# GuyTevet/motion-diffusion-model

Hardware: NVIDIA H100
Metric: motions/sec (higher is better)
Workload: dtype fp16 operands / fp32 accumulate (in/out projections hi-lo split)

## Files before the change

### motion-diffusion-model_b200/csrc/engine.cu

```cuda
#include <cuda.h>
#include <cuda_fp16.h>
#include <cuda_runtime.h>

#include <cmath>
#include <cstdarg>
#include <cstdio>
#include <cstring>
#include <map>
#include <string>
#include <vector>

#include "../../include/b200mdm.h"
#include "attention_tc.cuh"
#include "epilogues.cuh"
#include "gemm.cuh"
#include "gemm_ln.cuh"
#include "postprocess.cuh"
#include "kernels.cuh"

using namespace b200;

static thread_local char g_err[512] = "";
static int fail(int code, const char* fmt, ...) {
  va_list ap;
  va_start(ap, fmt);
  vsnprintf(g_err, sizeof(g_err), fmt, ap);
  va_end(ap);
  return code;
}
#define CUDA_TRY(expr)                                                                               \
  do {                                                                                               \
    cudaError_t _e = (expr);                                                                         \
    if (_e != cudaSuccess)                                                                           \
      return fail(B200MDM_ECUDA, "%s failed: %s (%s:%d)", #expr, cudaGetErrorString(_e), __FILE__, __LINE__); \
  } while (0)
#define TRY(expr)            \
  do {                       \
    int _r = (expr);         \
    if (_r != B200MDM_OK) return _r; \
  } while (0)

typedef CUresult (*EncodeTiledFn)(CUtensorMap*, CUtensorMapDataType, cuuint32_t, void*, const cuuint64_t*,
                                  const cuuint64_t*, const cuuint32_t*, const cuuint32_t*, CUtensorMapInterleave,
                                  CUtensorMapSwizzle, CUtensorMapL2promotion, CUtensorMapFloatOOBfill);
static EncodeTiledFn g_encode = nullptr;
static int resolve_driver() {
  if (g_encode) return B200MDM_OK;
  void* fn = nullptr;
  cudaDriverEntryPointQueryResult qres;
// ... 129 lines not shown
  std::vector<int> h_kv, h_action;
  std::vector<unsigned char> h_mask;
  bool dec = false;
  int ctx = 0, s_off = 1;
  int kw = 1;
  const unsigned char* inpaint_mask = nullptr;
  const float* inpaint_motion = nullptr;
  unsigned long long noise_seed = 0;
  long long noise_sample_base = 0;
  StepState* state = nullptr;
  cudaStream_t work = nullptr;
  cudaEvent_t ev_in = nullptr, ev_out = nullptr;
  long long launches = 0;
};

template <class T>
static int dalloc(T** p, size_t n, bool zero = false) {
  CUDA_TRY(cudaMalloc(reinterpret_cast<void**>(p), n * sizeof(T)));
  if (zero) CUDA_TRY(cudaMemset(*p, 0, n * sizeof(T)));
  return B200MDM_OK;
}
template <class T>
static void dfree(T*& p) {
  if (p) cudaFree(p);
  p = nullptr;
}

template <int BN, class Epi, bool RES = false>
static int set_gemm_attr() {
  CUDA_TRY(cudaFuncSetAttribute(gemm_f16_wgmma<BN, Epi, RES>, cudaFuncAttributeMaxDynamicSharedMemorySize,
                                GemmSmem<BN, Epi, RES>::TOTAL));
  return B200MDM_OK;
}
template <int KEYS>
static int set_attention_attr() {
  CUDA_TRY(cudaFuncSetAttribute(attention_tc_kernel<KEYS, false>, cudaFuncAttributeMaxDynamicSharedMemorySize,
                                AttnTcSmem::total(KEYS)));
  CUDA_TRY(cudaFuncSetAttribute(attention_tc_kernel<KEYS, true>, cudaFuncAttributeMaxDynamicSharedMemorySize,
                                AttnTcSmem::total(KEYS)));
  return B200MDM_OK;
}
static int init_kernel_attrs() {
  static unsigned long long done_mask = 0;
  int dev = 0;
  CUDA_TRY(cudaGetDevice(&dev));
  if (dev < 64 && ((done_mask >> dev) & 1ull)) return B200MDM_OK;
  TRY((set_gemm_attr<128, EpiBiasF16<false>>()));
  TRY((set_gemm_attr<128, EpiBiasF16<true>>()));
  TRY((set_gemm_attr<256, EpiBiasF16<false>>()));
  TRY((set_gemm_attr<256, EpiBiasF16<true>>()));
  TRY((set_gemm_attr<64, EpiBiasF16<false>, true>()));
  TRY((set_gemm_attr<64, EpiBiasF16<true>, true>()));
  TRY((set_gemm_attr<128, EpiBiasF16Wide<true>>()));
  TRY((set_gemm_attr<128, EpiBiasF16Global>()));
  CUDA_TRY(cudaFuncSetAttribute(gemm_resid_ln_cluster, cudaFuncAttributeMaxDynamicSharedMemorySize, GemmLnSmem::TOTAL));
  TRY((set_gemm_attr<128, EpiEmbed>()));
  TRY((set_gemm_attr<96, EpiOutStep>()));
  TRY((set_attention_attr<64>()));
  TRY((set_attention_attr<208>()));
  TRY((set_attention_attr<256>()));
  if (dev < 64) done_mask |= 1ull << dev;
  return B200MDM_OK;
}

static bool g_pdl_now = false;
static bool pdl_enabled() {
  static int v = -1;
  if (v < 0) {
    const char* e = getenv("B200MDM_PDL");
    v = (e && e[0] == '0') ? 0 : 1;
  }
  return v == 1;
}
struct PdlScope {
  PdlScope() { g_pdl_now = pdl_enabled(); }
  ~PdlScope() { g_pdl_now = false; }
};
template <class... KArgs, class... Args>
static cudaError_t launch_k(void (*kern)(KArgs...), dim3 grid, dim3 block, size_t smem, cudaStream_t s, Args&&... args) {
  cudaLaunchConfig_t cfg;
  memset(&cfg, 0, sizeof(cfg));
  cfg.gridDim = grid;
  cfg.blockDim = block;
  cfg.dynamicSmemBytes = smem;
  cfg.stream = s;
  cudaLaunchAttribute at[1];
  at[0].id = cudaLaunchAttributeProgrammaticStreamSerialization;
  at[0].val.programmaticStreamSerializationAllowed = 1;
  cfg.attrs = at;
  cfg.numAttrs = g_pdl_now ? 1 : 0;
  return cudaLaunchKernelEx(&cfg, kern, static_cast<KArgs>(std::forward<Args>(args))...);
}

template <int BN, class Epi, class = void> struct epi_unstaged : std::false_type {};
template <int BN, class Epi> struct epi_unstaged<BN, Epi, std::enable_if_t<Epi::UNSTAGED>> : std::true_type {};

template <int BN, class Epi>
static int launch_gemm(const CUtensorMap& a, const CUtensorMap& b, const CUtensorMap& c, int M, int N, int K,
                       const typename Epi::Params& p, cudaStream_t s, int num_sms) {
  if (!epi_unstaged<BN, Epi>::value && N * 4 > GEMM_BIAS_BYTES)
    return fail(B200MDM_ENOTIMPL, "GEMM epilogue vectors are staged for N <= %d", GEMM_BIAS_BYTES / 4);
  const int tiles = ((M + GEMM_BLOCK_M - 1) / GEMM_BLOCK_M) * ((N + BN - 1) / BN);
  const int grid = tiles < num_sms ? tiles : num_sms;
  CUDA_TRY(launch_k(gemm_f16_wgmma<BN, Epi>, dim3(grid), dim3(GEMM_THREADS), GemmSmem<BN, Epi>::TOTAL, s, a, b, c, M, N, K, p));
  return B200MDM_OK;
}
template <int BN, class Epi>
static int launch_gemm_resident(const CUtensorMap& a, const CUtensorMap& b, const CUtensorMap& c, int M, int N, int K,
                                const typename Epi::Params& p, cudaStream_t s, int num_sms) {
  const int tiles_n = (N + BN - 1) / BN;
  const int tiles = ((M + GEMM_BLOCK_M - 1) / GEMM_BLOCK_M) * tiles_n;
  const int grid = tiles < num_sms ? tiles : num_sms;
  if (K > GEMM_RES_KB_MAX * GEMM_BLOCK_K || tiles_n > grid || N * 4 > GEMM_BIAS_BYTES)
    return fail(B200MDM_ENOTIMPL, "W-resident GEMM needs K <= %d and N <= %d", GEMM_RES_KB_MAX * GEMM_BLOCK_K, grid * BN);
  CUDA_TRY(launch_k(gemm_f16_wgmma<BN, Epi, true>, dim3(grid), dim3(GEMM_THREADS), GemmSmem<BN, Epi, true>::TOTAL, s, a, b, c, M, N, K, p));
  return B200MDM_OK;
}
template <bool GELU>
static int launch_gemm_bias(const CUtensorMap& a, const CUtensorMap& b, const CUtensorMap& c, int M, int N, int K,
                            const float* bias, cudaStream_t s, int num_sms) {
  typename EpiBiasF16<GELU>::Params p{bias};
  return launch_gemm<128, EpiBiasF16<GELU>>(a, b, c, M, N, K, p, s, num_sms);
}

static int launch_gemm_resid_ln(const CUtensorMap& a, const CUtensorMap& w256, const CUtensorMap& hres, int M, int K,
                                const float* bias, const float* gamma, const float* beta, cudaStream_t s, int num_sms) {
  const int tiles = (M + GEMM_BLOCK_M - 1) / GEMM_BLOCK_M;
  const int max_clusters = num_sms / 2;
  const int clusters = tiles < max_clusters ? tiles : max_clusters;
  GemmLnParams lp{bias, gamma, beta, 1e-5f};
  CUDA_TRY(launch_k(gemm_resid_ln_cluster, dim3(2 * clusters), dim3(GLN_THREADS), GemmLnSmem::TOTAL, s, a, w256, hres, M, K, lp));
  return B200MDM_OK;
}

static int make_attention_kv_map(CUtensorMap* m, const void* qkv, int n_samples, int S, int ld) {
  return make_map_3d(m, qkv, n_samples, S, ld, ld, atc_keys(S));
}
template <int KEYS>
static cudaError_t launch_attention_keys(const CUtensorMap& map_kv, const __half* qkv, __half* out, const int* kvlen,
                                         dim3 grid, int S, int d, float scale_log2, cudaStream_t s, bool wide) {
  return launch_k(wide ? attention_tc_kernel<KEYS, true> : attention_tc_kernel<KEYS, false>, grid, dim3(ATC_THREADS),
                  AttnTcSmem::total(KEYS), s, map_kv, qkv, out, kvlen, S, d, scale_log2);
}
static int launch_attention_tc(const CUtensorMap& map_kv, const __half* qkv, __half* out, const int* kvlen, int n_samples,
                               int S, int d, int H, cudaStream_t s, bool wide = false) {
  if (d != H * ATC_DH) return fail(B200MDM_ENOTIMPL, "attention: head_dim must be 128");
  if (S > ATC_MAX_KEYS) return fail(B200MDM_ENOTIMPL, "attention: at most %d tokens per sample", ATC_MAX_KEYS);
  const float scale_log2 = 1.4426950408889634f / sqrtf(static_cast<float>(ATC_DH));
  const int tiles = (S + ATC_QROWS - 1) / ATC_QROWS;
  const dim3 grid(H, n_samples, (tiles + ATC_TILES_PER_CTA - 1) / ATC_TILES_PER_CTA);
  const int keys = atc_keys(S);
  if (keys == 64) CUDA_TRY(launch_attention_keys<64>(map_kv, qkv, out, kvlen, grid, S, d, scale_log2, s, wide));
  else if (keys == 208) CUDA_TRY(launch_attention_keys<208>(map_kv, qkv, out, kvlen, grid, S, d, scale_log2, s, wide));
  else CUDA_TRY(launch_attention_keys<256>(map_kv, qkv, out, kvlen, grid, S, d, scale_log2, s, wide));
  return B200MDM_OK;
// ... 651 lines not shown

static int enqueue_forward(b200mdm_engine* e, const StepArgs& a, cudaStream_t s, int* n_kernels) {
  const int d = e->d, ff = e->ff, B = e->B, T = e->T, S = e->S, JF = e->JF, Kp = e->Kp_in;
  int nk = 0;
  PdlScope pdl_scope;
  if (a.philox) {
    const long long quads = (static_cast<long long>(JF) * T + 3) / 4 * B;
    const int blocks = static_cast<int>(quads / 256 + 1 < 1184 ? quads / 256 + 1 : 1184);
    CUDA_TRY(launch_k(philox_normal_kernel, dim3(blocks), dim3(256), 0, s, e->eps_buf, B, static_cast<long long>(JF) * T,
                      0ull, 0ll, 0u, e->state));
    ++nk;
  }
  {
    dim3 grid((T + 31) / 32, (JF + 31) / 32, B), block(32, 8);
    CUDA_TRY(launch_k(pack_input_kernel, grid, block, 0, s, a.x_in, e->xin16, B, JF, T, S, Kp, 3 * Kp, e->s_off));
    ++nk;
  }
  {
    EpiEmbed::Params p;
    p.res_c = e->m_res_c; p.res_u = e->m_res_u;
    p.pe_bias = e->pe_bias;
    p.S = S; p.d = d; p.halves = e->halves;
    TRY((launch_gemm<128, EpiEmbed>(e->m_xin, e->m_win, e->m_xin, e->MB, d, 3 * Kp, p, s, e->num_sms)));
    ++nk;
  }
  const float* target_g = e->target_set ? e->tgt_g : nullptr;
  if (!e->dec) {
    CUDA_TRY(launch_k(tok0_rows_kernel, dim3(e->Bp), dim3(128), 0, s, e->hres, e->condproj, e->temb_table, e->pe,
                      a.explicit_t ? e->tvec : nullptr, e->tmap, e->state, target_g, B, S, d, e->cfg.temb_rows));
  } else {
    CUDA_TRY(launch_k(mem_build_kernel, dim3(e->Mt, e->Bp), dim3(128), 0, s, e->mem16, e->memproj, e->temb_table,
                      a.explicit_t ? e->tvec : nullptr, e->tmap, e->state, target_g, B, e->Mt, d, e->cfg.temb_rows));
    EpiBiasF16Global::Params p{e->bkv_all};
    TRY((launch_gemm<128, EpiBiasF16Global>(e->m_mem, e->m_wkv_all, e->m_kvc_st, e->Bp * e->Mt, e->L * 2 * d, d, p, s, e->num_sms)));
    ++nk;
  }
  ++nk;
  const int kw = e->kw;
  const bool wide = kw == 2;
  for (int l = 0; l < e->L; ++l) {
    const LayerW& w = e->layers[l];
    if (B200_SKIP(1)) {
      ++nk;
    } else {
      {
        TRY((launch_gemm_bias<false>(e->m_h16, w.m_wqkv, e->m_qkv_st, e->M, 3 * d, d, w.bqkv, s, e->num_sms)));
      }
      TRY(launch_attention_tc(e->m_qkv_kv, e->qkv16, e->att16, e->kvlen, e->Bp, S, d, e->H, s, wide));
    }
    if (!B200_SKIP(2)) TRY(launch_gemm_resid_ln(e->m_att, w.m_wo_256, e->m_hres, e->M, kw * d, w.bo, w.g1, w.be1, s, e->num_sms));
    if (e->dec) {
      TRY((launch_gemm_bias<false>(e->m_h16, w.m_wq_c, e->m_qc_st, e->M, d, d, w.bq_c, s, e->num_sms)));
      {
        const float sl2 = 1.4426950408889634f / sqrtf(128.0f);
        const dim3 cg(e->H, e->Bp), cb(128);
        const __half* kvl = e->kvc16 + static_cast<size_t>(l) * 2 * d;
        const int ldkv = e->L * 2 * d;
        if (e->Mt <= 16)
          CUDA_TRY(launch_k(cross_attention_kernel<2>, cg, cb, 0, s, e->qc16, kvl, e->memmask, e->att16, S, e->Mt, d, ldkv, sl2));
        else if (e->Mt <= 32)
          CUDA_TRY(launch_k(cross_attention_kernel<4>, cg, cb, 0, s, e->qc16, kvl, e->memmask, e->att16, S, e->Mt, d, ldkv, sl2));
        else
          CUDA_TRY(launch_k(cross_attention_kernel<8>, cg, cb, 0, s, e->qc16, kvl, e->memmask, e->att16, S, e->Mt, d, ldkv, sl2));
      }
      TRY(launch_gemm_resid_ln(e->m_att, w.m_wo_c_256, e->m_hres, e->M, d, w.bo_c, w.g2, w.be2, s, e->num_sms));
      nk += 3;
    }
    if (wide) {
      EpiBiasF16Wide<true>::Params p{w.b1, ff};
      TRY((launch_gemm<128, EpiBiasF16Wide<true>>(e->m_h16, w.m_w1, e->m_ffn_st, e->M, ff, kw * d, p, s, e->num_sms)));
    } else if (!B200_SKIP(4)) {
      TRY((launch_gemm_bias<true>(e->m_h16, w.m_w1, e->m_ffn_st, e->M, ff, d, w.b1, s, e->num_sms)));
    }
    if (!B200_SKIP(8)) TRY(launch_gemm_resid_ln(e->m_ffn, w.m_w2_256, e->m_hres, e->M, kw * ff, w.b2, e->dec ? w.g3 : w.g2,
                             e->dec ? w.be3 : w.be2, s, e->num_sms));
    nk += 5;
  }
  CUDA_TRY(launch_k(blend_split_kernel, dim3((B * T + 7) / 8), dim3(256), 0, s, e->hres, e->g16, e->scale, B, S, T, e->s_off, d,
                    e->halves));
  ++nk;
  {
    EpiOutStep::Params p;
    p.bias = e->b_out;
    p.x_t = a.x_in;
    p.noise = a.noise;
    p.x_out = a.x_out;
    p.pred_xstart = a.pred;
    p.inpaint_mask = e->inpaint_mask;
    p.inpaint_motion = e->inpaint_motion;
    p.sched = e->sched;
    p.state = e->state;
    p.noise_batch_stride = a.const_noise ? 0 : static_cast<long long>(JF) * T;
    p.B = B; p.S = T; p.T = T; p.J = JF; p.mode = a.mode;
    p.s_off = 0;
    p.clip_denoised = a.clip;
    TRY((launch_gemm<96, EpiOutStep>(e->m_g16, e->m_wout, e->m_g16, B * T, e->N_out_pad, 3 * d, p, s, e->num_sms)));
    ++nk;
  }
  *n_kernels = nk;
  return B200MDM_OK;
}

static int check_ready(b200mdm_engine* e, bool need_sched) {
// ... 157 lines not shown
  CUDA_TRY(cudaGetLastError());
  return B200MDM_OK;
}

extern "C" int b200mdm_q_sample(b200mdm_engine* e, float sqrt_ac, float sqrt_1mac, const float* x_start_dev,
                                const float* noise_dev, float* out_dev, int64_t n, void* stream) {
  if (!e || !noise_dev || !out_dev || n <= 0) return fail(B200MDM_EINVAL, "bad argument");
  q_sample_kernel<<<592, 256, 0, static_cast<cudaStream_t>(stream)>>>(out_dev, x_start_dev, noise_dev, sqrt_ac, sqrt_1mac,
                                                                     static_cast<size_t>(n));
  CUDA_TRY(cudaGetLastError());
  e->launches++;
  return B200MDM_OK;
}

extern "C" int64_t b200mdm_launch_count(b200mdm_engine* e, int32_t reset) {
  if (!e) return 0;
  long long v = e->launches;
  if (reset) e->launches = 0;
  return v;
}

template <int BN, bool RES = false>
static int test_gemm_bn(const void* a16, const void* w16, const float* bias, void* out16, int M, int N, int K, int act,
                        cudaStream_t s, int sms) {
  CUtensorMap ma, mb, mc;
  TRY(make_map(&ma, a16, M, K, K, GEMM_BLOCK_M));
  TRY(make_map(&mb, w16, N, K, K, BN));
  TRY(make_map_t(&mc, out16, 2, M, N, N, 32));
  EpiBiasF16<true>::Params pg{bias};
  EpiBiasF16<false>::Params pn{bias};
  if constexpr (RES)
    return act ? launch_gemm_resident<BN, EpiBiasF16<true>>(ma, mb, mc, M, N, K, pg, s, sms)
               : launch_gemm_resident<BN, EpiBiasF16<false>>(ma, mb, mc, M, N, K, pn, s, sms);
  else
    return act ? launch_gemm<BN, EpiBiasF16<true>>(ma, mb, mc, M, N, K, pg, s, sms)
               : launch_gemm<BN, EpiBiasF16<false>>(ma, mb, mc, M, N, K, pn, s, sms);
}

extern "C" int b200mdm_test_gemm_f16(const void* a16_dev, const void* w16_dev, const float* bias_dev, void* out16_dev,
                                     int32_t M, int32_t N, int32_t K, int32_t act, int32_t block_n, void* stream) {
  if (!a16_dev || !w16_dev || !bias_dev || !out16_dev || M <= 0 || N <= 0 || K <= 0 || K % 8 || N % 8)
    return fail(B200MDM_EINVAL, "bad argument (K %% 8 == 0, N %% 8 == 0 required)");
  TRY(init_kernel_attrs());
  int dev = 0, sms = 132;
  CUDA_TRY(cudaGetDevice(&dev));
  CUDA_TRY(cudaDeviceGetAttribute(&sms, cudaDevAttrMultiProcessorCount, dev));
  cudaStream_t s = static_cast<cudaStream_t>(stream);
  if (block_n == 128) return test_gemm_bn<128>(a16_dev, w16_dev, bias_dev, out16_dev, M, N, K, act, s, sms);
  if (block_n == 512) return test_gemm_bn<256>(a16_dev, w16_dev, bias_dev, out16_dev, M, N, K, act, s, sms);
  if (block_n == 513) return test_gemm_bn<64, true>(a16_dev, w16_dev, bias_dev, out16_dev, M, N, K, act, s, sms);
  return fail(B200MDM_EINVAL, "block_n must be 128 (128 x 128 tiles), 512 (128 x 256 tiles) or 513 (W-resident, 128 x 64 tiles)");
}

struct StreamScratch {
  cudaStream_t s;
  std::vector<void*> ptrs;
  explicit StreamScratch(cudaStream_t st) : s(st) {}
  ~StreamScratch() {
    for (void* p : ptrs) cudaFreeAsync(p, s);
  }
  template <class T>
  int alloc(T** p, size_t n, bool zero = false) {
    CUDA_TRY(cudaMallocAsync(reinterpret_cast<void**>(p), n * sizeof(T), s));
    ptrs.push_back(*p);
    if (zero) CUDA_TRY(cudaMemsetAsync(*p, 0, n * sizeof(T), s));
    return B200MDM_OK;
  }
};

static int device_sms(int* sms) {
  int dev = 0;
  CUDA_TRY(cudaGetDevice(&dev));
  CUDA_TRY(cudaDeviceGetAttribute(sms, cudaDevAttrMultiProcessorCount, dev));
  return B200MDM_OK;
}

extern "C" int b200mdm_test_gemm_epi(const void* a16_dev, const void* w16_dev, const float* bias_dev, void* out16_dev,
                                     int32_t M, int32_t N, int32_t K, int32_t epi, void* stream) {
  if (!a16_dev || !w16_dev || !bias_dev || !out16_dev || M <= 0 || N <= 0 || K <= 0 || K % 8)
    return fail(B200MDM_EINVAL, "bad argument (K %% 8 == 0 required)");
  TRY(init_kernel_attrs());
  int sms = 132;
  TRY(device_sms(&sms));
  cudaStream_t s = static_cast<cudaStream_t>(stream);
  CUtensorMap ma, mb, mc;
  TRY(make_map(&ma, a16_dev, M, K, K, GEMM_BLOCK_M));
  TRY(make_map(&mb, w16_dev, N, K, K, 128));
  if (epi == 0) {
    if (N % 64) return fail(B200MDM_EINVAL, "EpiBiasF16Wide needs N %% 64 == 0");
    TRY(make_map_t(&mc, out16_dev, 2, M, 2 * static_cast<uint64_t>(N), 2 * static_cast<uint64_t>(N), 32));
    EpiBiasF16Wide<true>::Params p{bias_dev, N};
    return launch_gemm<128, EpiBiasF16Wide<true>>(ma, mb, mc, M, N, K, p, s, sms);
  }
  if (epi == 1) {
    if (N % 32) return fail(B200MDM_EINVAL, "EpiBiasF16Global needs N %% 32 == 0");
    TRY(make_map_t(&mc, out16_dev, 2, M, N, N, 32));
    EpiBiasF16Global::Params p{bias_dev};
    return launch_gemm<128, EpiBiasF16Global>(ma, mb, mc, M, N, K, p, s, sms);
  }
  return fail(B200MDM_EINVAL, "epi must be 0 (EpiBiasF16Wide<GELU>) or 1 (EpiBiasF16Global)");
}

extern "C" int b200mdm_test_embed(const float* x_dev, const float* w_in_dev, const float* b_in_dev, const float* pe_dev,
                                  void* hres16_dev, int32_t B, int32_t JF, int32_t T, int32_t d, int32_t s_off,
                                  int32_t halves, void* stream) {
  if (!x_dev || !w_in_dev || !b_in_dev || !pe_dev || !hres16_dev || B <= 0 || JF <= 0 || T <= 0 || s_off < 0 ||
      d <= 0 || d % 64 || d * 4 > GEMM_BIAS_BYTES || (halves != 1 && halves != 2))
    return fail(B200MDM_EINVAL, "bad argument (d %% 64 == 0, d <= %d, halves 1 or 2)", GEMM_BIAS_BYTES / 4);
  TRY(init_kernel_attrs());
  int sms = 132;
  TRY(device_sms(&sms));
  cudaStream_t s = static_cast<cudaStream_t>(stream);
  const int S = T + s_off, Kp = (JF + 7) & ~7, MB = B * S;
  StreamScratch scr(s);
  __half *xin16 = nullptr, *w_in3 = nullptr;
  float* pe_bias = nullptr;
  TRY(scr.alloc(&xin16, static_cast<size_t>(MB) * 3 * Kp, true));
  TRY(scr.alloc(&w_in3, static_cast<size_t>(d) * 3 * Kp, true));
  TRY(scr.alloc(&pe_bias, static_cast<size_t>(S) * d));
  {
    dim3 grid((T + 31) / 32, (JF + 31) / 32, B), block(32, 8);
    pack_input_kernel<<<grid, block, 0, s>>>(x_dev, xin16, B, JF, T, S, Kp, 3 * Kp, s_off);
    CUDA_TRY(cudaGetLastError());
  }
  split_weight_kernel<<<d, 128, 0, s>>>(w_in_dev, w_in3, d, JF, Kp);
  CUDA_TRY(cudaGetLastError());
  pe_bias_kernel<<<S, 128, 0, s>>>(pe_bias, pe_dev, b_in_dev, S, d);
  CUDA_TRY(cudaGetLastError());
  CUtensorMap m_xin, m_win;
  TRY(make_map(&m_xin, xin16, MB, 3 * Kp, 3 * Kp, GEMM_BLOCK_M));
  TRY(make_map(&m_win, w_in3, d, 3 * Kp, 3 * Kp, 128));
// ... 161 lines not shown
```

### motion-diffusion-model_b200/csrc/epilogues.cuh

```cuda
#pragma once
#include <cuda_fp16.h>

#include "gemm.cuh"
#include "ptx.cuh"

namespace b200 {

__device__ __forceinline__ uint32_t slab_off(int r, int j) { return r * 128 + ((j ^ (r & 7)) << 4); }
__device__ __forceinline__ uint32_t slab64_off(int r, int j) { return r * 64 + ((j ^ ((r >> 1) & 3)) << 4); }

__device__ __forceinline__ void split_hi_lo8(const float (&v)[8], uint32_t (&hi)[4], uint32_t (&lo)[4]) {
#pragma unroll
  for (int i = 0; i < 4; ++i) {
    const __half2 h = __floats2half2_rn(v[2 * i], v[2 * i + 1]);
    const float2 f = __half22float2(h);
    const __half2 l = __floats2half2_rn(v[2 * i] - f.x, v[2 * i + 1] - f.y);
    hi[i] = *reinterpret_cast<const uint32_t*>(&h);
    lo[i] = *reinterpret_cast<const uint32_t*>(&l);
  }
}
__device__ __forceinline__ void join_hi_lo8(const uint4& h, const uint4& l, float (&v)[8]) {
  const uint32_t hw[4] = {h.x, h.y, h.z, h.w}, lw[4] = {l.x, l.y, l.z, l.w};
#pragma unroll
  for (int i = 0; i < 4; ++i) {
// ... 65 lines not shown
      __syncwarp();
    }
    uint32_t pk[16];
#pragma unroll
    for (int j = 0; j < 32; j += 4) {
      const float4 b = *reinterpret_cast<const float4*>(bs + j);
      float x0 = __uint_as_float(raw[j + 0]) + b.x, x1 = __uint_as_float(raw[j + 1]) + b.y;
      float x2 = __uint_as_float(raw[j + 2]) + b.z, x3 = __uint_as_float(raw[j + 3]) + b.w;
      if (GELU) {
        x0 = gelu_erf(x0); x1 = gelu_erf(x1); x2 = gelu_erf(x2); x3 = gelu_erf(x3);
      }
      pk[j / 2] = pack_half2(x0, x1);
      pk[j / 2 + 1] = pack_half2(x2, x3);
    }
#pragma unroll
    for (int j = 0; j < 4; ++j)
      *reinterpret_cast<uint4*>(slab + slab_off(ctx.lane, half * 4 + j)) =
          make_uint4(pk[4 * j], pk[4 * j + 1], pk[4 * j + 2], pk[4 * j + 3]);
    if (half == 1 || col0 + 32 >= ctx.N) {
      fence_proxy_async_smem();
      __syncwarp();
      if (ctx.lane == 0) {
        tma_store_2d(ctx.map_c, slab, col0 - 32 * half, row0);
        bulk_commit_group();
      }
      ctx.seq++;
    }
  }
  static __device__ __forceinline__ void tile_end(EpiCtx&, const Params&, int, int) {}
  static __device__ __forceinline__ void finish(EpiCtx& ctx) {
    if (ctx.lane == 0) bulk_wait_group<0>();
    __syncwarp();
  }
};

struct EpiBiasF16Global : EpiBiasF16<false> {
  static constexpr bool UNSTAGED = true;
  static __device__ __forceinline__ void preload(const Params&, float*, int, int, int) {}
  static __device__ __forceinline__ void chunk(EpiCtx& ctx, const Params& p, uint32_t (&raw)[32], int row0, int col0, int) {
    chunk_bias(ctx, p.bias + col0, raw, row0, col0);
  }
};

template <bool GELU>
struct EpiBiasF16Wide {
  static constexpr int SMEM_PER_WARP = 2 * 4096;
  struct Params {
    const float* bias;
    int lo_col;
  };
  static __device__ __forceinline__ void preload(const Params& p, float* dst, int N, int tid, int nthreads) {
    for (int i = tid; i < N; i += nthreads) dst[i] = p.bias[i];
  }
  static __device__ __forceinline__ void tile_begin(EpiCtx&, const Params&, int, int) {}
  static __device__ __forceinline__ void chunk(EpiCtx& ctx, const Params& p, uint32_t (&raw)[32], int row0, int col0,
                                               int) {
    const int half = (col0 >> 5) & 1;
    uint8_t* slab_hi = ctx.smem;
    uint8_t* slab_lo = ctx.smem + 4096;
    if (half == 0) {
      if (ctx.lane == 0) bulk_wait_group_read<0>();
      __syncwarp();
    }
    const float* bs = ctx.bias_all + col0;
#pragma unroll
    for (int j = 0; j < 4; ++j) {
      uint32_t hi[4], lo[4];
#pragma unroll
      for (int i = 0; i < 4; ++i) {
        float x0 = __uint_as_float(raw[8 * j + 2 * i]) + bs[8 * j + 2 * i];
        float x1 = __uint_as_float(raw[8 * j + 2 * i + 1]) + bs[8 * j + 2 * i + 1];
        if (GELU) {
          x0 = gelu_erf(x0); x1 = gelu_erf(x1);
        }
        const __half2 h = __floats2half2_rn(x0, x1);
        const float2 f = __half22float2(h);
        const __half2 l = __floats2half2_rn(x0 - f.x, x1 - f.y);
        hi[i] = *reinterpret_cast<const uint32_t*>(&h);
        lo[i] = *reinterpret_cast<const uint32_t*>(&l);
      }
      *reinterpret_cast<uint4*>(slab_hi + slab_off(ctx.lane, half * 4 + j)) = make_uint4(hi[0], hi[1], hi[2], hi[3]);
      *reinterpret_cast<uint4*>(slab_lo + slab_off(ctx.lane, half * 4 + j)) = make_uint4(lo[0], lo[1], lo[2], lo[3]);
    }
    if (half == 1 || col0 + 32 >= ctx.N) {
      fence_proxy_async_smem();
      __syncwarp();
      if (ctx.lane == 0) {
        tma_store_2d(ctx.map_c, slab_hi, col0 - 32 * half, row0);
        tma_store_2d(ctx.map_c, slab_lo, p.lo_col + col0 - 32 * half, row0);
        bulk_commit_group();
      }
      ctx.seq++;
    }
  }
  static __device__ __forceinline__ void tile_end(EpiCtx&, const Params&, int, int) {}
  static __device__ __forceinline__ void finish(EpiCtx& ctx) {
    if (ctx.lane == 0) bulk_wait_group<0>();
    __syncwarp();
  }
};

struct EpiEmbed {
  static constexpr int SMEM_PER_WARP = 2 * 4096;
  template <class P> static __device__ __forceinline__ void preload(const P&, float*, int, int, int) {}
  struct Params {
    CUtensorMap res_c, res_u;
    const float* pe_bias;
    int S, d, halves;
  };
  static __device__ __forceinline__ void tile_begin(EpiCtx&, const Params&, int, int) {}
  static __device__ __forceinline__ void chunk(EpiCtx& ctx, const Params& p, uint32_t (&raw)[32], int row0, int col0,
                                               int) {
    uint8_t* slab = ctx.smem + (ctx.seq & 1) * 4096;
    if (ctx.lane == 0) bulk_wait_group_read<1>();
    __syncwarp();
    const int row = row0 + ctx.lane;
    const int s = (row < ctx.M) ? row % p.S : 0;
    const float* pb = p.pe_bias + static_cast<size_t>(s) * p.d + col0;
#pragma unroll
    for (int j = 0; j < 4; ++j) {
      const float4 a0 = __ldg(reinterpret_cast<const float4*>(pb + 8 * j));
      const float4 a1 = __ldg(reinterpret_cast<const float4*>(pb + 8 * j + 4));
      const float o[8] = {__uint_as_float(raw[8 * j + 0]) + a0.x, __uint_as_float(raw[8 * j + 1]) + a0.y,
                          __uint_as_float(raw[8 * j + 2]) + a0.z, __uint_as_float(raw[8 * j + 3]) + a0.w,
                          __uint_as_float(raw[8 * j + 4]) + a1.x, __uint_as_float(raw[8 * j + 5]) + a1.y,
                          __uint_as_float(raw[8 * j + 6]) + a1.z, __uint_as_float(raw[8 * j + 7]) + a1.w};
      uint32_t hi[4], lo[4];
      split_hi_lo8(o, hi, lo);
      *reinterpret_cast<uint4*>(slab + slab64_off(ctx.lane, j)) = make_uint4(hi[0], hi[1], hi[2], hi[3]);
      *reinterpret_cast<uint4*>(slab + 2048 + slab64_off(ctx.lane, j)) = make_uint4(lo[0], lo[1], lo[2], lo[3]);
    }
// ... 107 lines not shown
```

### motion-diffusion-model_b200/csrc/ptx.cuh

```cuda
#pragma once
#include <cuda.h>
#include <cuda_fp16.h>
#include <cuda_runtime.h>
#include <stdint.h>

namespace b200 {

__device__ __forceinline__ uint32_t smem_u32(const void* p) {
  return static_cast<uint32_t>(__cvta_generic_to_shared(p));
}

__device__ __forceinline__ bool elect_one() {
  uint32_t pred = 0;
  asm volatile(
      "{\n\t.reg .pred P;\n\t"
      "elect.sync _|P, 0xffffffff;\n\t"
      "selp.u32 %0, 1, 0, P;\n\t}\n"
      : "=r"(pred));
  return pred != 0;
}

__device__ __forceinline__ void mbar_init(uint64_t* bar, uint32_t count) {
  asm volatile("mbarrier.init.shared::cta.b64 [%0], %1;" ::"r"(smem_u32(bar)), "r"(count) : "memory");
}
// ... 39 lines not shown
__device__ __forceinline__ void tma_prefetch_desc(const CUtensorMap* m) {
  asm volatile("prefetch.tensormap [%0];" ::"l"(reinterpret_cast<uint64_t>(m)) : "memory");
}
__device__ __forceinline__ void tma_load_2d(void* smem_dst, const CUtensorMap* map, uint64_t* bar, int c0, int c1) {
  asm volatile(
      "cp.async.bulk.tensor.2d.shared::cluster.global.mbarrier::complete_tx::bytes [%0], [%1, {%3, %4}], [%2];"
      ::"r"(smem_u32(smem_dst)), "l"(reinterpret_cast<uint64_t>(map)), "r"(smem_u32(bar)), "r"(c0), "r"(c1)
      : "memory");
}
__device__ __forceinline__ void tma_load_3d(void* smem_dst, const CUtensorMap* map, uint64_t* bar, int c0, int c1, int c2) {
  asm volatile(
      "cp.async.bulk.tensor.3d.shared::cluster.global.mbarrier::complete_tx::bytes [%0], [%1, {%3, %4, %5}], [%2];"
      ::"r"(smem_u32(smem_dst)), "l"(reinterpret_cast<uint64_t>(map)), "r"(smem_u32(bar)), "r"(c0), "r"(c1), "r"(c2)
      : "memory");
}
__device__ __forceinline__ void tma_store_2d(const CUtensorMap* map, const void* smem_src, int c0, int c1) {
  asm volatile("cp.async.bulk.tensor.2d.global.shared::cta.bulk_group [%0, {%2, %3}], [%1];"
               ::"l"(reinterpret_cast<uint64_t>(map)), "r"(smem_u32(smem_src)), "r"(c0), "r"(c1)
               : "memory");
}
__device__ __forceinline__ void bulk_commit_group() { asm volatile("cp.async.bulk.commit_group;" ::: "memory"); }
template <int N>
__device__ __forceinline__ void bulk_wait_group_read() {
  asm volatile("cp.async.bulk.wait_group.read %0;" ::"n"(N) : "memory");
}
template <int N>
__device__ __forceinline__ void bulk_wait_group() {
  asm volatile("cp.async.bulk.wait_group %0;" ::"n"(N) : "memory");
}

__device__ __forceinline__ void named_bar_sync(int id, int nthreads) {
  asm volatile("bar.sync %0, %1;" ::"r"(id), "r"(nthreads) : "memory");
}

__device__ __forceinline__ void pdl_wait() { asm volatile("griddepcontrol.wait;" ::: "memory"); }
__device__ __forceinline__ void pdl_launch_dependents() { asm volatile("griddepcontrol.launch_dependents;" ::: "memory"); }

__device__ __forceinline__ uint32_t cluster_ctarank() {
  uint32_t r;
  asm volatile("mov.u32 %0, %%cluster_ctarank;" : "=r"(r));
  return r;
}
__device__ __forceinline__ uint32_t mapa_shared(uint32_t local_smem_addr, uint32_t cta_rank) {
  uint32_t r;
  asm volatile("mapa.shared::cluster.u32 %0, %1, %2;" : "=r"(r) : "r"(local_smem_addr), "r"(cta_rank));
  return r;
}
__device__ __forceinline__ bool mbar_try_wait_cluster(uint64_t* bar, uint32_t parity) {
  uint32_t ok;
  asm volatile(
      "{\n\t.reg .pred P;\n\t"
      "mbarrier.try_wait.parity.acquire.cluster.shared::cta.b64 P, [%1], %2;\n\t"
      "selp.u32 %0, 1, 0, P;\n\t}\n"
      : "=r"(ok)
      : "r"(smem_u32(bar)), "r"(parity)
      : "memory");
  return ok != 0;
}
__device__ __forceinline__ void mbar_wait_cluster(uint64_t* bar, uint32_t parity) {
  if (mbar_try_wait_cluster(bar, parity)) return;
  long long t0 = clock64();
  while (!mbar_try_wait_cluster(bar, parity)) {
    if (clock64() - t0 > B200_WATCHDOG_CYCLES) __trap();
  }
}
__device__ __forceinline__ void cluster_sync_all() {
// ... 56 lines not shown
```

Measured before the change: 356.7.

## Add ping-pong warpgroup GEMM kernel for BN=128 bias, wide and global epilogues

Introduces a new ping-pong persistent GEMM in which the two consumer warpgroups each own whole 128x128 tiles and alternate, so one warpgroup's epilogue runs while the other issues WGMMA on the next tile. All BN=128 bias/GELU, hi-lo wide, and global-bias GEMM launches are routed to it, and the epilogues gain per-pair hooks that write into swizzled smem slabs followed by TMA stores. This aims to hide epilogue cost (GELU, hi-lo split, stores) behind tensor-core work. In exchange, each warpgroup now holds 128 accumulator registers, and the tile turn-taking relies on named barriers.

Result: faster. 378.3, median of 6 (+6.1%).

```diff
diff --git a/motion-diffusion-model_b200/csrc/engine.cu b/motion-diffusion-model_b200/csrc/engine.cu
--- a/motion-diffusion-model_b200/csrc/engine.cu
+++ b/motion-diffusion-model_b200/csrc/engine.cu
@@ -15,6 +15,7 @@
 #include "epilogues.cuh"
 #include "gemm.cuh"
 #include "gemm_ln.cuh"
+#include "gemm_pingpong.cuh"
 #include "postprocess.cuh"
 #include "kernels.cuh"
 
@@ -210,6 +211,11 @@
                                 GemmSmem<BN, Epi, RES>::TOTAL));
   return B200MDM_OK;
 }
+template <class Epi>
+static int set_pingpong_attr() {
+  CUDA_TRY(cudaFuncSetAttribute(gemm_f16_pingpong<Epi>, cudaFuncAttributeMaxDynamicSharedMemorySize, PP_SMEM_BYTES));
+  return B200MDM_OK;
+}
 template <int KEYS>
 static int set_attention_attr() {
   CUDA_TRY(cudaFuncSetAttribute(attention_tc_kernel<KEYS, false>, cudaFuncAttributeMaxDynamicSharedMemorySize,
@@ -223,14 +229,14 @@
   int dev = 0;
   CUDA_TRY(cudaGetDevice(&dev));
   if (dev < 64 && ((done_mask >> dev) & 1ull)) return B200MDM_OK;
-  TRY((set_gemm_attr<128, EpiBiasF16<false>>()));
-  TRY((set_gemm_attr<128, EpiBiasF16<true>>()));
+  TRY((set_pingpong_attr<EpiBiasF16<false>>()));
+  TRY((set_pingpong_attr<EpiBiasF16<true>>()));
+  TRY((set_pingpong_attr<EpiBiasF16Wide<true>>()));
+  TRY((set_pingpong_attr<EpiBiasF16Global>()));
   TRY((set_gemm_attr<256, EpiBiasF16<false>>()));
   TRY((set_gemm_attr<256, EpiBiasF16<true>>()));
   TRY((set_gemm_attr<64, EpiBiasF16<false>, true>()));
   TRY((set_gemm_attr<64, EpiBiasF16<true>, true>()));
-  TRY((set_gemm_attr<128, EpiBiasF16Wide<true>>()));
-  TRY((set_gemm_attr<128, EpiBiasF16Global>()));
   CUDA_TRY(cudaFuncSetAttribute(gemm_resid_ln_cluster, cudaFuncAttributeMaxDynamicSharedMemorySize, GemmLnSmem::TOTAL));
   TRY((set_gemm_attr<128, EpiEmbed>()));
   TRY((set_gemm_attr<96, EpiOutStep>()));
@@ -294,11 +300,21 @@
   CUDA_TRY(launch_k(gemm_f16_wgmma<BN, Epi, true>, dim3(grid), dim3(GEMM_THREADS), GemmSmem<BN, Epi, true>::TOTAL, s, a, b, c, M, N, K, p));
   return B200MDM_OK;
 }
+template <class Epi>
+static int launch_gemm_pp(const CUtensorMap& a, const CUtensorMap& b, const CUtensorMap& c, int M, int N, int K,
+                          const typename Epi::Params& p, cudaStream_t s, int num_sms) {
+  if (!epi_unstaged<PP_BLOCK_N, Epi>::value && N * 4 > GEMM_BIAS_BYTES)
+    return fail(B200MDM_ENOTIMPL, "GEMM epilogue vectors are staged for N <= %d", GEMM_BIAS_BYTES / 4);
+  const int tiles = ((M + GEMM_BLOCK_M - 1) / GEMM_BLOCK_M) * ((N + PP_BLOCK_N - 1) / PP_BLOCK_N);
+  const int grid = tiles < num_sms ? tiles : num_sms;
+  CUDA_TRY(launch_k(gemm_f16_pingpong<Epi>, dim3(grid), dim3(GEMM_THREADS), PP_SMEM_BYTES, s, a, b, c, M, N, K, p));
+  return B200MDM_OK;
+}
 template <bool GELU>
 static int launch_gemm_bias(const CUtensorMap& a, const CUtensorMap& b, const CUtensorMap& c, int M, int N, int K,
                             const float* bias, cudaStream_t s, int num_sms) {
   typename EpiBiasF16<GELU>::Params p{bias};
-  return launch_gemm<128, EpiBiasF16<GELU>>(a, b, c, M, N, K, p, s, num_sms);
+  return launch_gemm_pp<EpiBiasF16<GELU>>(a, b, c, M, N, K, p, s, num_sms);
 }
 
 static int launch_gemm_resid_ln(const CUtensorMap& a, const CUtensorMap& w256, const CUtensorMap& hres, int M, int K,
@@ -1016,7 +1032,7 @@
     CUDA_TRY(launch_k(mem_build_kernel, dim3(e->Mt, e->Bp), dim3(128), 0, s, e->mem16, e->memproj, e->temb_table,
                       a.explicit_t ? e->tvec : nullptr, e->tmap, e->state, target_g, B, e->Mt, d, e->cfg.temb_rows));
     EpiBiasF16Global::Params p{e->bkv_all};
-    TRY((launch_gemm<128, EpiBiasF16Global>(e->m_mem, e->m_wkv_all, e->m_kvc_st, e->Bp * e->Mt, e->L * 2 * d, d, p, s, e->num_sms)));
+    TRY((launch_gemm_pp<EpiBiasF16Global>(e->m_mem, e->m_wkv_all, e->m_kvc_st, e->Bp * e->Mt, e->L * 2 * d, d, p, s, e->num_sms)));
     ++nk;
   }
   ++nk;
@@ -1052,7 +1068,7 @@
     }
     if (wide) {
       EpiBiasF16Wide<true>::Params p{w.b1, ff};
-      TRY((launch_gemm<128, EpiBiasF16Wide<true>>(e->m_h16, w.m_w1, e->m_ffn_st, e->M, ff, kw * d, p, s, e->num_sms)));
+      TRY((launch_gemm_pp<EpiBiasF16Wide<true>>(e->m_h16, w.m_w1, e->m_ffn_st, e->M, ff, kw * d, p, s, e->num_sms)));
     } else if (!B200_SKIP(4)) {
       TRY((launch_gemm_bias<true>(e->m_h16, w.m_w1, e->m_ffn_st, e->M, ff, d, w.b1, s, e->num_sms)));
     }
@@ -1276,6 +1292,9 @@
   if constexpr (RES)
     return act ? launch_gemm_resident<BN, EpiBiasF16<true>>(ma, mb, mc, M, N, K, pg, s, sms)
                : launch_gemm_resident<BN, EpiBiasF16<false>>(ma, mb, mc, M, N, K, pn, s, sms);
+  else if constexpr (BN == PP_BLOCK_N)
+    return act ? launch_gemm_pp<EpiBiasF16<true>>(ma, mb, mc, M, N, K, pg, s, sms)
+               : launch_gemm_pp<EpiBiasF16<false>>(ma, mb, mc, M, N, K, pn, s, sms);
   else
     return act ? launch_gemm<BN, EpiBiasF16<true>>(ma, mb, mc, M, N, K, pg, s, sms)
                : launch_gemm<BN, EpiBiasF16<false>>(ma, mb, mc, M, N, K, pn, s, sms);
@@ -1334,13 +1353,13 @@
     if (N % 64) return fail(B200MDM_EINVAL, "EpiBiasF16Wide needs N %% 64 == 0");
     TRY(make_map_t(&mc, out16_dev, 2, M, 2 * static_cast<uint64_t>(N), 2 * static_cast<uint64_t>(N), 32));
     EpiBiasF16Wide<true>::Params p{bias_dev, N};
-    return launch_gemm<128, EpiBiasF16Wide<true>>(ma, mb, mc, M, N, K, p, s, sms);
+    return launch_gemm_pp<EpiBiasF16Wide<true>>(ma, mb, mc, M, N, K, p, s, sms);
   }
   if (epi == 1) {
     if (N % 32) return fail(B200MDM_EINVAL, "EpiBiasF16Global needs N %% 32 == 0");
     TRY(make_map_t(&mc, out16_dev, 2, M, N, N, 32));
     EpiBiasF16Global::Params p{bias_dev};
-    return launch_gemm<128, EpiBiasF16Global>(ma, mb, mc, M, N, K, p, s, sms);
+    return launch_gemm_pp<EpiBiasF16Global>(ma, mb, mc, M, N, K, p, s, sms);
   }
   return fail(B200MDM_EINVAL, "epi must be 0 (EpiBiasF16Wide<GELU>) or 1 (EpiBiasF16Global)");
 }
diff --git a/motion-diffusion-model_b200/csrc/epilogues.cuh b/motion-diffusion-model_b200/csrc/epilogues.cuh
--- a/motion-diffusion-model_b200/csrc/epilogues.cuh
+++ b/motion-diffusion-model_b200/csrc/epilogues.cuh
@@ -121,19 +121,35 @@
     if (ctx.lane == 0) bulk_wait_group<0>();
     __syncwarp();
   }
+
+  static constexpr int PP_ROUND_COLS = 128;
+  static __device__ __forceinline__ const float* pp_tile_bias(const Params&, const float* bias_all, float*, int col_t, int, int) {
+    return bias_all + col_t;
+  }
+  static __device__ __forceinline__ void pp_pair(const Params&, float2 b, float a0, float a1, uint8_t* dst) {
+    float x0 = a0 + b.x, x1 = a1 + b.y;
+    if (GELU) {
+      x0 = gelu_erf(x0); x1 = gelu_erf(x1);
+    }
+    *reinterpret_cast<uint32_t*>(dst) = pack_half2(x0, x1);
+  }
+  static __device__ __forceinline__ void pp_store(const CUtensorMap* map_c, const Params&, const uint8_t* box, int col, int row) {
+    tma_store_2d(map_c, box, col, row);
+  }
 };
 
 struct EpiBiasF16Global : EpiBiasF16<false> {
   static constexpr bool UNSTAGED = true;
   static __device__ __forceinline__ void preload(const Params&, float*, int, int, int) {}
-  static __device__ __forceinline__ void chunk(EpiCtx& ctx, const Params& p, uint32_t (&raw)[32], int row0, int col0, int) {
-    chunk_bias(ctx, p.bias + col0, raw, row0, col0);
+  static __device__ __forceinline__ const float* pp_tile_bias(const Params& p, const float*, float* scratch, int col_t, int N,
+                                                              int tid) {
+    scratch[tid] = col_t + tid < N ? __ldg(p.bias + col_t + tid) : 0.f;
+    return scratch;
   }
 };
 
 template <bool GELU>
 struct EpiBiasF16Wide {
-  static constexpr int SMEM_PER_WARP = 2 * 4096;
   struct Params {
     const float* bias;
     int lo_col;
@@ -141,51 +157,24 @@
   static __device__ __forceinline__ void preload(const Params& p, float* dst, int N, int tid, int nthreads) {
     for (int i = tid; i < N; i += nthreads) dst[i] = p.bias[i];
   }
-  static __device__ __forceinline__ void tile_begin(EpiCtx&, const Params&, int, int) {}
-  static __device__ __forceinline__ void chunk(EpiCtx& ctx, const Params& p, uint32_t (&raw)[32], int row0, int col0,
-                                               int) {
-    const int half = (col0 >> 5) & 1;
-    uint8_t* slab_hi = ctx.smem;
-    uint8_t* slab_lo = ctx.smem + 4096;
-    if (half == 0) {
-      if (ctx.lane == 0) bulk_wait_group_read<0>();
-      __syncwarp();
-    }
-    const float* bs = ctx.bias_all + col0;
-#pragma unroll
-    for (int j = 0; j < 4; ++j) {
-      uint32_t hi[4], lo[4];
-#pragma unroll
-      for (int i = 0; i < 4; ++i) {
-        float x0 = __uint_as_float(raw[8 * j + 2 * i]) + bs[8 * j + 2 * i];
-        float x1 = __uint_as_float(raw[8 * j + 2 * i + 1]) + bs[8 * j + 2 * i + 1];
-        if (GELU) {
-          x0 = gelu_erf(x0); x1 = gelu_erf(x1);
-        }
-        const __half2 h = __floats2half2_rn(x0, x1);
-        const float2 f = __half22float2(h);
-        const __half2 l = __floats2half2_rn(x0 - f.x, x1 - f.y);
-        hi[i] = *reinterpret_cast<const uint32_t*>(&h);
-        lo[i] = *reinterpret_cast<const uint32_t*>(&l);
-      }
-      *reinterpret_cast<uint4*>(slab_hi + slab_off(ctx.lane, half * 4 + j)) = make_uint4(hi[0], hi[1], hi[2], hi[3]);
-      *reinterpret_cast<uint4*>(slab_lo + slab_off(ctx.lane, half * 4 + j)) = make_uint4(lo[0], lo[1], lo[2], lo[3]);
-    }
-    if (half == 1 || col0 + 32 >= ctx.N) {
-      fence_proxy_async_smem();
-      __syncwarp();
-      if (ctx.lane == 0) {
-        tma_store_2d(ctx.map_c, slab_hi, col0 - 32 * half, row0);
-        tma_store_2d(ctx.map_c, slab_lo, p.lo_col + col0 - 32 * half, row0);
-        bulk_commit_group();
-      }
-      ctx.seq++;
-    }
-  }
-  static __device__ __forceinline__ void tile_end(EpiCtx&, const Params&, int, int) {}
-  static __device__ __forceinline__ void finish(EpiCtx& ctx) {
-    if (ctx.lane == 0) bulk_wait_group<0>();
-    __syncwarp();
+  static constexpr int PP_ROUND_COLS = 64;
+  static __device__ __forceinline__ const float* pp_tile_bias(const Params&, const float* bias_all, float*, int col_t, int, int) {
+    return bias_all + col_t;
+  }
+  static __device__ __forceinline__ void pp_pair(const Params&, float2 b, float a0, float a1, uint8_t* dst) {
+    float x0 = a0 + b.x, x1 = a1 + b.y;
+    if (GELU) {
+      x0 = gelu_erf(x0); x1 = gelu_erf(x1);
+    }
+    const __half2 h = __floats2half2_rn(x0, x1);
+    const float2 f = __half22float2(h);
+    const __half2 l = __floats2half2_rn(x0 - f.x, x1 - f.y);
+    *reinterpret_cast<__half2*>(dst) = h;
+    *reinterpret_cast<__half2*>(dst + 16384) = l;
+  }
+  static __device__ __forceinline__ void pp_store(const CUtensorMap* map_c, const Params& p, const uint8_t* box, int col, int row) {
+    tma_store_2d(map_c, box, col, row);
+    tma_store_2d(map_c, box + 16384, p.lo_col + col, row);
   }
 };
 
diff --git a/motion-diffusion-model_b200/csrc/gemm_pingpong.cuh b/motion-diffusion-model_b200/csrc/gemm_pingpong.cuh
--- /dev/null
+++ b/motion-diffusion-model_b200/csrc/gemm_pingpong.cuh
@@ -0,0 +1,153 @@
+#pragma once
+#include "epilogues.cuh"
+#include "gemm.cuh"
+
+namespace b200 {
+
+constexpr int PP_BLOCK_N = 128;
+constexpr int PP_A_BYTES = GEMM_BLOCK_M * GEMM_BLOCK_K * 2;
+constexpr int PP_STAGE_BYTES = PP_A_BYTES + PP_BLOCK_N * GEMM_BLOCK_K * 2;
+constexpr int PP_SLAB_BYTES = 2 * GEMM_BLOCK_M * 128;
+constexpr int PP_STAGES = (227 * 1024 - 1024  - 2 * PP_SLAB_BYTES - GEMM_BIAS_BYTES - GEMM_BAR_BYTES) /
+                          PP_STAGE_BYTES;
+constexpr int PP_SMEM_BYTES = 1024 + PP_STAGES * PP_STAGE_BYTES + 2 * PP_SLAB_BYTES + GEMM_BIAS_BYTES + GEMM_BAR_BYTES;
+static_assert(PP_STAGES == 4, "shared-memory budget: 4 operand stages of 32 KB");
+constexpr int PP_BAR_TURN = 1, PP_BAR_EPI = 3;
+
+template <class Epi>
+__global__ void __launch_bounds__(GEMM_THREADS, 1)
+gemm_f16_pingpong(const __grid_constant__ CUtensorMap map_a, const __grid_constant__ CUtensorMap map_b,
+                  const __grid_constant__ CUtensorMap map_c, int M, int N, int K,
+                  const __grid_constant__ typename Epi::Params ep) {
+  constexpr int RC = Epi::PP_ROUND_COLS;
+  static_assert(RC == 64 || RC == 128, "a round is one or two 64-column slabs");
+
+  extern __shared__ uint8_t smem_raw[];
+  uint8_t* smem = smem_raw + ((1024u - (smem_u32(smem_raw) & 1023u)) & 1023u);
+  uint8_t* tiles = smem;
+  uint8_t* slabs = tiles + PP_STAGES * PP_STAGE_BYTES;
+  float* bias_all = reinterpret_cast<float*>(slabs + 2 * PP_SLAB_BYTES);
+  uint64_t* full_bar = reinterpret_cast<uint64_t*>(slabs + 2 * PP_SLAB_BYTES + GEMM_BIAS_BYTES);
+  uint64_t* empty_bar = full_bar + PP_STAGES;
+
+  const int warp = threadIdx.x >> 5;
+  const int lane = threadIdx.x & 31;
+  const int tiles_m = (M + GEMM_BLOCK_M - 1) / GEMM_BLOCK_M;
+  const int tiles_n = (N + PP_BLOCK_N - 1) / PP_BLOCK_N;
+  const int num_tiles = tiles_m * tiles_n;
+  const int num_kb = (K + GEMM_BLOCK_K - 1) / GEMM_BLOCK_K;
+  const int my_tiles = static_cast<int>(blockIdx.x) < num_tiles ? (num_tiles - 1 - blockIdx.x) / gridDim.x + 1 : 0;
+
+  pdl_launch_dependents();
+  Epi::preload(ep, bias_all, N, threadIdx.x, blockDim.x);
+  if (threadIdx.x == 0) {
+    tma_prefetch_desc(&map_a);
+    tma_prefetch_desc(&map_b);
+    tma_prefetch_desc(&map_c);
+    for (int s = 0; s < PP_STAGES; ++s) {
+      mbar_init(&full_bar[s], 1);
+      mbar_init(&empty_bar[s], 4);
+    }
+    fence_barrier_init();
+  }
+  __syncthreads();
+  pdl_wait();
+
+  if (warp < 4) {
+    asm volatile("setmaxnreg.dec.sync.aligned.u32 %0;" ::"n"(GEMM_REGS_PRODUCER));
+    if (warp == 0 && elect_one()) {
+      int stage = 0;
+      uint32_t phase = 0;
+      for (int i = 0; i < my_tiles; ++i) {
+        const int tile = blockIdx.x + i * gridDim.x;
+        const int m_blk = tile / tiles_n, n_blk = tile % tiles_n;
+        for (int kb = 0; kb < num_kb; ++kb) {
+          mbar_wait(&empty_bar[stage], phase ^ 1);
+          uint8_t* sa = tiles + stage * PP_STAGE_BYTES;
+          mbar_expect_tx(&full_bar[stage], PP_STAGE_BYTES);
+          tma_load_2d(sa, &map_a, &full_bar[stage], kb * GEMM_BLOCK_K, m_blk * GEMM_BLOCK_M);
+          tma_load_2d(sa + PP_A_BYTES, &map_b, &full_bar[stage], kb * GEMM_BLOCK_K, n_blk * PP_BLOCK_N);
+          if (++stage == PP_STAGES) { stage = 0; phase ^= 1; }
+        }
+      }
+    }
+  } else {
+    asm volatile("setmaxnreg.inc.sync.aligned.u32 %0;" ::"n"(GEMM_REGS_CONSUMER));
+    const int wg = (warp >> 2) - 1;
+    const int wq = warp & 3;
+    const int g = lane >> 2, t = lane & 3;
+    const bool leader = wq == 0 && lane == 0;
+    uint8_t* slab = slabs + wg * PP_SLAB_BYTES;
+    const int toff = (16 * wq + g) * 128 + 4 * t;
+    float acc0[64], acc1[64];
+    for (int i = wg; i < my_tiles; i += 2) {
+      const int tile = blockIdx.x + i * gridDim.x;
+      const int m_blk = tile / tiles_n, n_blk = tile % tiles_n;
+      const int pos = i * num_kb;
+      int stage = pos % PP_STAGES;
+      uint32_t phase = (pos / PP_STAGES) & 1;
+      if (i > 0) named_bar_sync(PP_BAR_TURN + wg, 256);
+      int prev_stage = -1;
+      for (int kb = 0; kb < num_kb; ++kb) {
+        mbar_wait(&full_bar[stage], phase);
+        const uint32_t sa = smem_u32(tiles + stage * PP_STAGE_BYTES);
+        const uint64_t da0 = wgmma_desc_k_sw128(sa);
+        const uint64_t da1 = wgmma_desc_k_sw128(sa + 64 * 128);
+        const uint64_t db = wgmma_desc_k_sw128(sa + PP_A_BYTES);
+        wgmma_fence_acc(acc0);
+        wgmma_fence_acc(acc1);
+        wgmma_fence();
+#pragma unroll
+        for (int k = 0; k < GEMM_BLOCK_K / 16; ++k) {
+          Wgmma<128>::mma(acc0, da0 + 2 * k, db + 2 * k, (kb | k) != 0);
+          Wgmma<128>::mma(acc1, da1 + 2 * k, db + 2 * k, (kb | k) != 0);
+        }
+        wgmma_commit();
+        wgmma_fence_acc(acc0);
+        wgmma_fence_acc(acc1);
+        wgmma_wait<1>();
+        if (prev_stage >= 0 && lane == 0) mbar_arrive(&empty_bar[prev_stage]);
+        prev_stage = stage;
+        if (++stage == PP_STAGES) { stage = 0; phase ^= 1; }
+      }
+      if (i + 1 < my_tiles) named_bar_arrive(PP_BAR_TURN + (wg ^ 1), 256);
+      wgmma_wait<0>();
+      wgmma_fence_acc(acc0);
+      wgmma_fence_acc(acc1);
+      if (lane == 0) mbar_arrive(&empty_bar[prev_stage]);
+      const int row_t = m_blk * GEMM_BLOCK_M, col_t = n_blk * PP_BLOCK_N;
+      const float* bs = Epi::pp_tile_bias(ep, bias_all, bias_all + wg * PP_BLOCK_N, col_t, N, threadIdx.x & 127);
+#pragma unroll
+      for (int c0 = 0; c0 < PP_BLOCK_N; c0 += RC) {
+        if (col_t + c0 >= N) break;
+        if (leader) bulk_wait_group_read<0>();
+        named_bar_sync(PP_BAR_EPI + wg, 128);
+#pragma unroll
+        for (int jj = 0; jj < RC / 8; ++jj) {
+          const int j = c0 / 8 + jj;
+          const float2 b = *reinterpret_cast<const float2*>(bs + 8 * j + 2 * t);
+          uint8_t* d = slab + (jj >> 3) * (GEMM_BLOCK_M * 128) + toff + (((jj & 7) ^ g) << 4);
+          Epi::pp_pair(ep, b, acc0[4 * j], acc0[4 * j + 1], d);
+          Epi::pp_pair(ep, b, acc0[4 * j + 2], acc0[4 * j + 3], d + 1024);
+          Epi::pp_pair(ep, b, acc1[4 * j], acc1[4 * j + 1], d + 8192);
+          Epi::pp_pair(ep, b, acc1[4 * j + 2], acc1[4 * j + 3], d + 8192 + 1024);
+        }
+        fence_proxy_async_smem();
+        named_bar_sync(PP_BAR_EPI + wg, 128);
+        if (leader) {
+#pragma unroll
+          for (int s = 0; s < RC / 64; ++s) {
+            const int col = col_t + c0 + 64 * s;
+            if (col < N)
+              for (int r = 0; r < GEMM_BLOCK_M; r += 32)
+                if (row_t + r < M) Epi::pp_store(&map_c, ep, slab + s * (GEMM_BLOCK_M * 128) + r * 128, col, row_t + r);
+          }
+          bulk_commit_group();
+        }
+      }
+    }
+    if (leader) bulk_wait_group<0>();
+  }
+}
+
+}
diff --git a/motion-diffusion-model_b200/csrc/ptx.cuh b/motion-diffusion-model_b200/csrc/ptx.cuh
--- a/motion-diffusion-model_b200/csrc/ptx.cuh
+++ b/motion-diffusion-model_b200/csrc/ptx.cuh
@@ -95,6 +95,9 @@
 __device__ __forceinline__ void named_bar_sync(int id, int nthreads) {
   asm volatile("bar.sync %0, %1;" ::"r"(id), "r"(nthreads) : "memory");
 }
+__device__ __forceinline__ void named_bar_arrive(int id, int nthreads) {
+  asm volatile("bar.arrive %0, %1;" ::"r"(id), "r"(nthreads) : "memory");
+}
 
 __device__ __forceinline__ void pdl_wait() { asm volatile("griddepcontrol.wait;" ::: "memory"); }
 __device__ __forceinline__ void pdl_launch_dependents() { asm volatile("griddepcontrol.launch_dependents;" ::: "memory"); }
```
